# jdm365/SuffixArray

Measured on AMD Instinct MI355X. Metric: sa_build_chars_per_s, higher is better.
Workload: dtype u8 text / u32 narrow keys / u32 suffix indices / i64 output

## Files before the change

suffixarray_amd/csrc/radix_narrow.hpp:

```cpp
#pragma once
#include "radix_sort.hpp"
#include <vector>

namespace sa {

constexpr int NARROW_MAX_PASSES = 6;
constexpr int SEG_ITEMS = 24;

struct SegPlan {
    u32 bstart[RADIX + 1];
    u32 tprefix[RADIX + 1];
    u32 cfirst[NCHUNK + 1];
};

__global__ __launch_bounds__(256) void seg_plan_kernel(const u32* __restrict__ hist_top, u32 tile, SegPlan* __restrict__ plan) {
    __shared__ u32 s_w[2][4];
    __shared__ u32 s_tp[RADIX + 1];
    const int d = threadIdx.x, lane = d & 63, w = d >> 6;
    u32 size = 0;
#pragma unroll
    for (int c = 0; c < NCHUNK; ++c) size += hist_top[c * RADIX + d];
    const u32 tiles = (u32)(((u64)size + tile - 1) / tile);
    u32 is = size, it = tiles;
#pragma unroll
// ... 767 lines not shown
    __syncthreads();
#pragma unroll
    for (int k = 0; k < ITEMS; ++k) {
        const u32 p = k * BLOCK + tid;
        if (FULL || p < tile_n) a.vals_out[gidx[k]] = s_vals[p];
    }
}

template <int BLOCK>
__global__ __launch_bounds__(BLOCK, 4) void text_low_pass_kernel(TextLowArgs t) {
    constexpr int WAVES = BLOCK / WAVE;
    constexpr u32 TILE = BLOCK * SORT_ITEMS;
    constexpr int WH = (WAVES * RADIX > NCHUNK * RADIX) ? WAVES * RADIX : NCHUNK * RADIX;
    static_assert(TILE * 8 >= TILE + TEXT_HALO, "the staged codes fit the key array's LDS");
    __shared__ __attribute__((aligned(16))) u64 s_keys[TILE];
    __shared__ u32 s_whist[WH];
    __shared__ uint2 s_tab[RADIX];
    __shared__ u32 s_wsum[RADIX / WAVE];
    __shared__ u8 s_map[256];
    __shared__ u32 s_tile;
    __shared__ u32 s_chunk;
    const SortPassArgs& a = t.p;
    const int tid = threadIdx.x;
    if (tid == 0) {
        u32 tile = 0xFFFFFFFFu, chunk = 0;
        const u32 home = xcc_id();
        for (int k = 0; k < NCHUNK; ++k) {
            const u32 c = (home + k) & (NCHUNK - 1);
            const u32 first = c * a.g.tpc;
            if (first >= a.g.tiles) continue;
            const u32 cnt = (a.g.tiles - first) < a.g.tpc ? (a.g.tiles - first) : a.g.tpc;
            const u32 x = atomicAdd(&a.ticket[c], 1u);
            if (x < cnt) { tile = first + x; chunk = c; break; }
        }
        s_tile = tile;
        s_chunk = chunk;
    }
    if (tid < 256) s_map[tid] = (u8)t.map[tid];
    for (int i = tid; i < WAVES * RADIX; i += BLOCK) s_whist[i] = 0;
    __syncthreads();
    const u32 tile = s_tile;
    if (tile == 0xFFFFFFFFu) return;
    const u32 chunk = s_chunk;
    const u64 rest = t.n - (u64)tile * TILE;
    if (rest >= (u64)TILE)
        text_low_tile<true, BLOCK>(t, tile, chunk, TILE, s_keys, s_whist, s_tab, s_wsum, s_map);
    else
        text_low_tile<false, BLOCK>(t, tile, chunk, (u32)rest, s_keys, s_whist, s_tab, s_wsum, s_map);
}

struct NarrowWorkspace {
    SegPlan* plan = nullptr;
    u32* hist = nullptr;
    u32* base = nullptr;
    u32* tickets = nullptr;
    u16* map_dev = nullptr;
    CodeMap map_host;
    bool split_enabled = true;
    bool split_used = false;
    u32 split_max_seen = 0;
    u32* split_hist = nullptr;
    u32* split_base = nullptr;
    u32* split_cursor = nullptr;
    u32* top_cursor = nullptr;
    bool cursor_pad = true;
    bool split_cursor_t = false;
    bool top_atomic_ranks = false;
    bool top_claims = true;
    bool split_atomic = true;
    u32* split_sub = nullptr;
    u64* split_status = nullptr;
    u32 split_tiles = 0;
    u32 split_epoch = 0;
    u32* host_word = nullptr;
    static size_t split_table_bytes() { return (size_t)RADIX * SPLIT_NB * sizeof(u32); }
    static size_t split_sub_words() { return ((size_t)RADIX << SPLIT_BITS) + 1; }
    u32* split_levels_dev() const { return split_sub + split_sub_words(); }
    u32 split_cap = LOCAL_CAP;
    int split_rb = 0;
    int local_bin_bits = 12;
    bool split_flags = true;
    bool local_big = false;
    bool split_big = false;
    bool split_flags_done = false;
    int split_items = 28;
    static size_t hist_bytes() { return (size_t)NARROW_MAX_PASSES * RADIX * RADIX * sizeof(u32); }
    int init() {
        SA_HIP_CHECK(hipMalloc(&plan, sizeof(SegPlan)));
        SA_HIP_CHECK(hipMalloc(&hist, hist_bytes()));
        SA_HIP_CHECK(hipMalloc(&base, (size_t)RADIX * RADIX * sizeof(u32)));
        SA_HIP_CHECK(hipMalloc(&tickets, (size_t)NARROW_MAX_PASSES * NCHUNK * sizeof(u32)));
        SA_HIP_CHECK(hipMalloc(&map_dev, sizeof(CodeMap)));
        SA_HIP_CHECK(hipMalloc(&split_hist, split_table_bytes()));
        SA_HIP_CHECK(hipMalloc(&split_base, split_table_bytes()));
        SA_HIP_CHECK(hipMalloc(&split_cursor, split_table_bytes()));
        SA_HIP_CHECK(hipMalloc(&top_cursor, (size_t)RADIX * 64 * sizeof(u32)));
        SA_HIP_CHECK(hipMalloc(&split_sub, (split_sub_words() + 16) * sizeof(u32)));
        SA_HIP_CHECK(hipHostMalloc(reinterpret_cast<void**>(&host_word), 64, hipHostMallocDefault));
        if (const char* e = diag_env("SA_HIP_SPLIT")) split_enabled = atoi(e) != 0;
        if (const char* e = diag_env("SA_HIP_CURSOR_PAD")) cursor_pad = atoi(e) != 0;
        if (const char* e = diag_env("SA_HIP_SPLIT_CURSOR_T")) split_cursor_t = atoi(e) != 0;
        if (const char* e = diag_env("SA_HIP_TOP_CLAIMS")) top_claims = atoi(e) != 0;
        if (const char* e = diag_env("SA_HIP_TOP_ARANKS")) top_atomic_ranks = atoi(e) != 0;
        if (const char* e = diag_env("SA_HIP_LOCAL_BIG")) local_big = atoi(e) != 0;
        if (const char* e = diag_env("SA_HIP_SPLIT_ATOMIC")) split_atomic = atoi(e) != 0;
        if (const char* e = diag_env("SA_HIP_SPLIT_FLAGS")) split_flags = atoi(e) != 0;
        if (const char* e = diag_env("SA_HIP_LOCAL_BINS")) local_bin_bits = (atoi(e) == 11) ? 11 : 12;
        if (const char* e = diag_env("SA_HIP_SPLIT_ITEMS")) { const int v = atoi(e); split_items = (v == 24 || v == 28) ? v : 32; }
        if (const char* e = diag_env("SA_HIP_SPLIT_CAP")) { const int v = atoi(e); if (v >= 64 && v <= (int)LOCAL_CAP) split_cap = (u32)v; }
        return 0;
    }
    int ensure_split_status(u32 tiles, hipStream_t stream) {
        if (tiles <= split_tiles) return 0;
        if (split_status) { SA_HIP_CHECK(hipStreamSynchronize(stream)); (void)hipFree(split_status); }
        split_status = nullptr; split_tiles = 0;
        SA_HIP_CHECK(hipMalloc(&split_status, (size_t)tiles * SPLIT_NB * sizeof(u64)));
        SA_HIP_CHECK(hipMemsetAsync(split_status, 0, (size_t)tiles * SPLIT_NB * sizeof(u64), stream));
        split_tiles = tiles;
        return 0;
    }
    void destroy() {
        if (plan) (void)hipFree(plan);
        if (hist) (void)hipFree(hist);
        if (base) (void)hipFree(base);
        if (tickets) (void)hipFree(tickets);
        if (map_dev) (void)hipFree(map_dev);
        if (split_hist) (void)hipFree(split_hist);
        if (split_base) (void)hipFree(split_base);
        if (split_cursor) (void)hipFree(split_cursor);
        if (top_cursor) (void)hipFree(top_cursor);
        if (split_sub) (void)hipFree(split_sub);
        if (split_status) (void)hipFree(split_status);
        if (host_word) (void)hipHostFree(host_word);
        map_dev = nullptr;
        plan = nullptr; hist = nullptr; base = nullptr; tickets = nullptr;
        split_hist = split_base = split_sub = split_cursor = top_cursor = nullptr; split_status = nullptr; split_tiles = 0; host_word = nullptr;
    }
};

inline bool narrow_sort_applies(const RadixWorkspace& ws, u64 n, int begin_bit) {
    return ws.block == 512 && begin_bit >= 24 && begin_bit < 56 && n >= (1u << 22) &&
           n / ws.tile() + RADIX + 1 <= ws.max_tiles;
}

struct TextSource {
    const u8* text;
    int b, k0;
};
inline bool text_pass_applies(int b, int k0) { return b <= 8 && k0 - 1 <= TEXT_HALO; }

inline int narrow_text_histogram(RadixWorkspace& ws, NarrowWorkspace& nw, hipStream_t stream, const u8* text, const CodeMap& map,
                                 u32 n, int b) {
    nw.map_host = map;
    SA_HIP_CHECK(hipMemcpyAsync(nw.map_dev, nw.map_host.code, sizeof(CodeMap), hipMemcpyHostToDevice, stream));
    const SortGeom g = make_geom(n, TEXT_TILE);
    const u32 spans = div_up(n, 4096);
    const dim3 grid(spans < 2048u ? spans : 2048u), block(256);
    switch ((8 + b - 1) / b) {
        case 1: hipLaunchKernelGGL(top_hist_kernel<1>, grid, block, 0, stream, text, nw.map_dev, (u64)n, b, g, ws.hist(0)); break;
        case 2: hipLaunchKernelGGL(top_hist_kernel<2>, grid, block, 0, stream, text, nw.map_dev, (u64)n, b, g, ws.hist(0)); break;
        case 3: hipLaunchKernelGGL(top_hist_kernel<3>, grid, block, 0, stream, text, nw.map_dev, (u64)n, b, g, ws.hist(0)); break;
        case 4: hipLaunchKernelGGL(top_hist_kernel<4>, grid, block, 0, stream, text, nw.map_dev, (u64)n, b, g, ws.hist(0)); break;
        default: hipLaunchKernelGGL(top_hist_kernel<8>, grid, block, 0, stream, text, nw.map_dev, (u64)n, b, g, ws.hist(0)); break;
    }
    return 0;
}

inline int wide_text_histogram(RadixWorkspace& ws, NarrowWorkspace& nw, hipStream_t stream, const u8* text, const CodeMap& map,
                               u32 n, int b, int k0) {
    nw.map_host = map;
    SA_HIP_CHECK(hipMemcpyAsync(nw.map_dev, nw.map_host.code, sizeof(CodeMap), hipMemcpyHostToDevice, stream));
    const SortGeom g = make_geom(n, ws.tile());
    const u32 spans = div_up(n, 4096);
    const dim3 grid(spans < 2048u ? spans : 2048u), block(256);
    switch ((8 + b - 1) / b) {
        case 1: hipLaunchKernelGGL(top_hist_kernel<1>, grid, block, 0, stream, text, nw.map_dev, (u64)n, b, g, ws.hist(0), k0); break;
        case 2: hipLaunchKernelGGL(top_hist_kernel<2>, grid, block, 0, stream, text, nw.map_dev, (u64)n, b, g, ws.hist(0), k0); break;
        case 3: hipLaunchKernelGGL(top_hist_kernel<3>, grid, block, 0, stream, text, nw.map_dev, (u64)n, b, g, ws.hist(0), k0); break;
        case 4: hipLaunchKernelGGL(top_hist_kernel<4>, grid, block, 0, stream, text, nw.map_dev, (u64)n, b, g, ws.hist(0), k0); break;
        default: hipLaunchKernelGGL(top_hist_kernel<8>, grid, block, 0, stream, text, nw.map_dev, (u64)n, b, g, ws.hist(0), k0); break;
    }
    return 0;
}
struct WideTextCtx {
    const u8* text;
    const u16* map;
    u64 n;
// ... 60 lines not shown
    const u32 split_flat_max = n / split_tile_n + 1 + RADIX;
    hipLaunchKernelGGL(seg_plan_kernel, dim3(1), dim3(256), 0, stream, ws.hist(0), try_split ? split_tile_n : seg_tile_n, nw.plan);
    nw.split_used = false;
    nw.split_flags_done = false;
    nw.split_max_seen = 0;
    if (try_split) {
        const int hb = (lo_bits - LOCAL_BIN_BITS < SPLIT_BITS) ? lo_bits - LOCAL_BIN_BITS : SPLIT_BITS;
        SA_HIP_CHECK(hipMemsetAsync(nw.split_hist, 0, NarrowWorkspace::split_table_bytes(), stream));
        SA_HIP_CHECK(hipMemsetAsync(nw.split_levels_dev(), 0, 16 * sizeof(u32), stream));
        const u32 tpb = 4;
        if (nw.split_items == 32)
            hipLaunchKernelGGL((split_hist_kernel<512, 32>), dim3(div_up(split_flat_max, tpb)), dim3(512), 0, stream,
                               reinterpret_cast<const u32*>(keysB), nw.plan, lo_bits - hb, (1u << hb) - 1u, nw.split_hist, tpb);
        else if (nw.split_items == 28)
            hipLaunchKernelGGL((split_hist_kernel<512, 28>), dim3(div_up(split_flat_max, tpb)), dim3(512), 0, stream,
                               reinterpret_cast<const u32*>(keysB), nw.plan, lo_bits - hb, (1u << hb) - 1u, nw.split_hist, tpb);
        else
            hipLaunchKernelGGL((split_hist_kernel<512, 24>), dim3(div_up(split_flat_max, tpb)), dim3(512), 0, stream,
                               reinterpret_cast<const u32*>(keysB), nw.plan, lo_bits - hb, (1u << hb) - 1u, nw.split_hist, tpb);
        hipLaunchKernelGGL(split_levels_kernel, dim3(RADIX), dim3(SPLIT_NB), 0, stream, (const u32*)nw.split_hist, hb, nw.split_levels_dev());
        SA_HIP_CHECK(hipMemcpyAsync(nw.host_word, nw.split_levels_dev(), 16 * sizeof(u32), hipMemcpyDeviceToHost, stream));
        SA_HIP_CHECK(hipStreamSynchronize(stream));
        int rb = -1;
        bool big = nw.local_big;
        if (!big)
            for (int k = 1; k <= hb; ++k)
                if (nw.host_word[k] <= nw.split_cap) { rb = k; break; }
        if (rb < 0 && nw.split_cap == LOCAL_CAP) {
            for (int k = 1; k <= hb; ++k)
                if (nw.host_word[k] <= LOCAL_CAP_BIG && lo_bits - k >= 12) { rb = k; big = true; break; }
            if (rb < 0) big = false;
        }
        nw.split_max_seen = nw.host_word[rb > 0 ? rb : hb];
        if (rb > 0) {
            const int rest_bits = lo_bits - rb;
            const int dshift = lo_bits - rb;
            const u32 dmask = (1u << rb) - 1u;
            hipLaunchKernelGGL(split_scan_kernel, dim3(RADIX), dim3(SPLIT_NB), 0, stream, (const u32*)nw.split_hist, nw.plan, hb, rb,
                               nw.split_base, nw.split_sub);
            if (!nw.split_atomic && (rc = nw.ensure_split_status(split_flat_max, stream))) return rc;
            if (nw.split_atomic) SA_HIP_CHECK(hipMemsetAsync(nw.split_cursor, 0, NarrowWorkspace::split_table_bytes(), stream));
            if (++ws.epoch >= (1u << 30)) {
                SA_HIP_CHECK(hipMemsetAsync(ws.status, 0, (size_t)ws.max_tiles * RADIX * sizeof(u64), stream));
                ws.epoch = 1;
            }
            if (!nw.split_atomic && ws.epoch <= nw.split_epoch)
                SA_HIP_CHECK(hipMemsetAsync(nw.split_status, 0, (size_t)nw.split_tiles * SPLIT_NB * sizeof(u64), stream));
            nw.split_epoch = ws.epoch;
            SplitPassArgs a;
            a.keys_in = reinterpret_cast<const u32*>(keysB); a.vals_in = valsB;
            a.keys_out = reinterpret_cast<u32*>(keysA); a.vals_out = valsA;
            a.plan = nw.plan; a.shift = dshift; a.mask = dmask; a.digit_base = nw.split_base; a.status = nw.split_status;
            a.ticket = nw.tickets; a.epoch = ws.epoch; a.dstat = ws.dstat; a.incl_mask = SA_INCL_MASK; a.cursor = nw.split_cursor;
            a.cur_bs = nw.split_cursor_t ? 1u : (u32)SPLIT_NB; a.cur_ds = nw.split_cursor_t ? (u32)RADIX : 1u;
            if ((rc = ws.timer.start(stream, 2))) return rc;
            if (nw.split_atomic) {
                if (nw.split_items == 32) hipLaunchKernelGGL((seg_split_kernel<512, 32, true>), dim3(split_flat_max), dim3(512), 0, stream, a);
                else if (nw.split_items == 28) hipLaunchKernelGGL((seg_split_kernel<512, 28, true>), dim3(split_flat_max), dim3(512), 0, stream, a);
                else hipLaunchKernelGGL((seg_split_kernel<512, 24, true>), dim3(split_flat_max), dim3(512), 0, stream, a);
            } else {
                if (nw.split_items == 32) hipLaunchKernelGGL((seg_split_kernel<512, 32, false>), dim3(split_flat_max), dim3(512), 0, stream, a);
                else if (nw.split_items == 28) hipLaunchKernelGGL((seg_split_kernel<512, 28, false>), dim3(split_flat_max), dim3(512), 0, stream, a);
                else hipLaunchKernelGGL((seg_split_kernel<512, 24, false>), dim3(split_flat_max), dim3(512), 0, stream, a);
            }
            if ((rc = ws.timer.stop(stream, (u64)n * 16u))) return rc;
            ws.pass_records += n; ws.pass_bytes += (u64)n * 16u; ws.passes += 1;
            LocalArgs l;
            l.keys_in = reinterpret_cast<const u32*>(keysA); l.vals_in = valsA;
            l.keys_out = reinterpret_cast<u32*>(keysB); l.vals_out = valsB; l.vals_out64 = vals_res64;
            l.sub = nw.split_sub;
            const int bb = (big || (rest_bits >= 12 && nw.local_bin_bits == 12)) ? 12 : 11;
            l.bin_shift = rest_bits - bb;
            l.dstat = ws.dstat;
            const u64 local_bytes = (u64)n * 16u + (vals_res64 ? (u64)n * 8u : 0u);
            nw.split_flags_done = false;
            l.dir = DirArgs{}; l.counts = nullptr; l.lite = LiteArgs{}; l.lo_shift = begin_bit; l.rb = rb; l.n = n;
            bool with_flags = false;
            if (nw.split_flags && flags_req && flags_req->prepare) {
                const int fr = flags_req->prepare(flags_req->ctx, (u32)RADIX << rb, &l);
                if (fr < 0) return fr;
                with_flags = (fr == 0) && l.dir.dir && l.dir.dbits >= 8 + rb && l.dir.dbits - 8 - rb <= bb && l.dir.dbits - 8 <= lo_bits;
            }
            if ((rc = ws.timer.start(stream, 3))) return rc;
            const dim3 lgrid((u32)RADIX << rb), lblock(big ? LOCAL_BLOCK_BIG : LOCAL_BLOCK);
            if (big) {
                if (with_flags) hipLaunchKernelGGL((local_finish_kernel<12, true, LOCAL_BLOCK_BIG>), lgrid, lblock, 0, stream, l);
                else hipLaunchKernelGGL((local_finish_kernel<12, false, LOCAL_BLOCK_BIG>), lgrid, lblock, 0, stream, l);
            } else if (with_flags) {
                if (bb == 12) hipLaunchKernelGGL((local_finish_kernel<12, true>), lgrid, lblock, 0, stream, l);
                else hipLaunchKernelGGL((local_finish_kernel<11, true>), lgrid, lblock, 0, stream, l);
            } else {
                if (bb == 12) hipLaunchKernelGGL((local_finish_kernel<12, false>), lgrid, lblock, 0, stream, l);
                else hipLaunchKernelGGL((local_finish_kernel<11, false>), lgrid, lblock, 0, stream, l);
            }
            nw.split_flags_done = with_flags;
            nw.split_big = big;
            if ((rc = ws.timer.stop(stream, local_bytes))) return rc;
            ws.pass_records += n; ws.pass_bytes += local_bytes; ws.passes += 1;
            SA_HIP_CHECK(hipGetLastError());
            if (diag_env("SA_HIP_SPLIT_DEBUG")) {
                const u32 nsub = (u32)RADIX << rb;
                std::vector<u32> sub(nsub + 1), k1(n), k2(n), v2(n), bst(RADIX + 1);
                SA_HIP_CHECK(hipStreamSynchronize(stream));
                SA_HIP_CHECK(hipMemcpy(sub.data(), nw.split_sub, (size_t)(nsub + 1) * 4, hipMemcpyDeviceToHost));
                SA_HIP_CHECK(hipMemcpy(k1.data(), keysA, (size_t)n * 4, hipMemcpyDeviceToHost));
                SA_HIP_CHECK(hipMemcpy(k2.data(), keysB, (size_t)n * 4, hipMemcpyDeviceToHost));
                SA_HIP_CHECK(hipMemcpy(v2.data(), valsB, (size_t)n * 4, hipMemcpyDeviceToHost));
                SA_HIP_CHECK(hipMemcpy(bst.data(), nw.plan->bstart, (size_t)(RADIX + 1) * 4, hipMemcpyDeviceToHost));
                u64 bad_sub = 0, bad_split = 0, bad_sorted = 0, bad_mono = 0;
                u32 first_split = ~0u, first_sorted = ~0u;
                for (u32 i = 0; i < nsub; ++i) {
                    if (sub[i] > sub[i + 1] || sub[i + 1] > n) { ++bad_mono; continue; }
                    if ((i & (((u32)1 << rb) - 1)) == 0 && sub[i] != bst[i >> rb]) ++bad_sub;
                    for (u32 j = sub[i]; j < sub[i + 1]; ++j) {
                        if (((k1[j] >> dshift) & dmask) != (i & dmask)) { ++bad_split; if (first_split == ~0u) first_split = j; }
                        if (j > sub[i] && (k2[j - 1] > k2[j] || (k2[j - 1] == k2[j] && v2[j - 1] >= v2[j]))) { ++bad_sorted; if (first_sorted == ~0u) first_sorted = j; }
                    }
                }
                fprintf(stderr, "[sa_hip] split debug: n=%u rb=%d hb=%d nsub=%u sub[0]=%u sub[last]=%u | table: %llu not monotone, %llu off the bucket starts | split pass: %llu records in the wrong group (first %u) | local pass: %llu out of order (first %u)\n",
                        n, rb, hb, nsub, sub[0], sub[nsub], (unsigned long long)bad_mono, (unsigned long long)bad_sub, (unsigned long long)bad_split, first_split,
                        (unsigned long long)bad_sorted, first_sorted);
            }
            nw.split_used = true;
            nw.split_rb = rb;
            *keys_res = reinterpret_cast<u64*>(keysB);
            *vals_res = valsB;
            return 0;
        }
    }
    if (optimistic) {
        SA_HIP_CHECK(hipMemsetAsync(ws.tickets(), 0, NCHUNK * sizeof(u32), stream));
        if (++ws.epoch >= (1u << 30)) {
            SA_HIP_CHECK(hipMemsetAsync(ws.status, 0, (size_t)ws.max_tiles * RADIX * sizeof(u64), stream));
            ws.epoch = 1;
        }
        if ((rc = launch_text_top(false))) return rc;
    }
    if (try_split && split_tile_n != seg_tile_n)
        hipLaunchKernelGGL(seg_plan_kernel, dim3(1), dim3(256), 0, stream, ws.hist(0), seg_tile_n, nw.plan);
    SA_HIP_CHECK(hipMemsetAsync(nw.hist, 0, NarrowWorkspace::hist_bytes(), stream));
    {
        const u32 tpb = 4;
        const u32 mask0 = (1u << ((np == 1) ? lo_bits : RADIX_BITS)) - 1u;
        hipLaunchKernelGGL((seg_hist_kernel<512, SEG_ITEMS>), dim3(div_up(flat_max, tpb)), dim3(512), 0, stream,
                           reinterpret_cast<const u32*>(keysB), nw.plan, 0, mask0, nw.hist, tpb);
    }
    u32* kin = reinterpret_cast<u32*>(keysB); u32* vin = valsB;
    u32* kout = reinterpret_cast<u32*>(keysA); u32* vout = valsA;
    for (int p = 0; p < np; ++p) {
        if (++ws.epoch >= (1u << 30)) {
            SA_HIP_CHECK(hipMemsetAsync(ws.status, 0, (size_t)ws.max_tiles * RADIX * sizeof(u64), stream));
            ws.epoch = 1;
        }
        const bool last = (p == np - 1);
        const int bits_p = last ? (lo_bits - RADIX_BITS * (np - 1)) : RADIX_BITS;
        hipLaunchKernelGGL(seg_scan_kernel, dim3(RADIX), dim3(256), 0, stream, nw.hist + (size_t)p * RADIX * RADIX, nw.plan, nw.base);
        SegPassArgs a;
        a.keys_in = kin; a.vals_in = vin; a.keys_out = kout; a.keys_out64 = keep_narrow ? nullptr : reinterpret_cast<u64*>(kout);
        a.vals_out = vout;
        a.vals_out64 = last ? vals_res64 : nullptr;
        a.plan = nw.plan;
        a.shift = RADIX_BITS * p;
        a.mask = (1u << bits_p) - 1u;
        a.next_shift = last ? -1 : RADIX_BITS * (p + 1);
        const int bits_n = (p + 1 == np - 1) ? (lo_bits - RADIX_BITS * (np - 1)) : RADIX_BITS;
        a.next_mask = last ? 0u : ((1u << bits_n) - 1u);
        a.digit_base = nw.base;
        a.next_hist = last ? nullptr : nw.hist + (size_t)(p + 1) * RADIX * RADIX;
// ... 19 lines not shown
```

suffixarray_amd/csrc/radix_split.hpp:

```cpp
#pragma once
#include "flags_common.hpp"

namespace sa {

#ifndef SA_ABL
#define SA_ABL 0
#endif
constexpr int SPLIT_BITS = 10;
constexpr int SPLIT_NB = 1 << SPLIT_BITS;
constexpr u32 LOCAL_CAP = 8192;
constexpr int LOCAL_BLOCK = 512;
constexpr int LOCAL_ITEMS = (int)(LOCAL_CAP / LOCAL_BLOCK);
constexpr u32 LOCAL_CAP_BIG = 16384;
constexpr int LOCAL_BLOCK_BIG = 1024;
constexpr int LOCAL_BIN_BITS = 11;
constexpr int SPLIT_HIST_COPIES = 4;

template <int BLOCK, int ITEMS>
__global__ __launch_bounds__(BLOCK) void split_hist_kernel(const u32* __restrict__ keys, const SegPlan* __restrict__ plan, int shift,
                                                           u32 mask, u32* __restrict__ hist, u32 tiles_per_block) {
    constexpr u32 TILE = BLOCK * ITEMS;
    constexpr int CS = SPLIT_NB + 1;
    __shared__ u32 s_h[SPLIT_HIST_COPIES * CS];
    __shared__ u32 s_t[RADIX + 1];
    for (int i = threadIdx.x; i <= RADIX; i += BLOCK) s_t[i] = plan->tprefix[i];
    for (int i = threadIdx.x; i < SPLIT_HIST_COPIES * CS; i += BLOCK) s_h[i] = 0;
    __syncthreads();
    const u32 F = s_t[RADIX];
    const u32 f_lo = blockIdx.x * tiles_per_block;
    const u32 f_hi = (f_lo + tiles_per_block < F) ? f_lo + tiles_per_block : F;
    if (f_lo >= f_hi) return;
    u32* my = s_h + (threadIdx.x & (SPLIT_HIST_COPIES - 1)) * CS;
    auto flush = [&](u32 bucket) {
        sync_lds();
        for (int d = threadIdx.x; d < SPLIT_NB; d += BLOCK) {
            u32 v = 0;
#pragma unroll
            for (int k = 0; k < SPLIT_HIST_COPIES; ++k) { v += s_h[k * CS + d]; s_h[k * CS + d] = 0; }
            if (v) atomicAdd(&hist[bucket * SPLIT_NB + d], v);
        }
        sync_lds();
    };
    u32 cur = seg_bucket_of(s_t, f_lo);
    for (u32 f = f_lo; f < f_hi; ++f) {
        const u32 b = seg_bucket_of(s_t, f);
        if (b != cur) { flush(cur); cur = b; }
        const u32 start = plan->bstart[b] + ((f - s_t[b]) * TILE);
        const u32 end = plan->bstart[b + 1];
        const u32 len = (end - start) < TILE ? (end - start) : TILE;
        if (len == TILE) {
            u32 k[ITEMS];
#pragma unroll
            for (int j = 0; j < ITEMS; ++j) k[j] = keys[start + j * BLOCK + threadIdx.x];
#pragma unroll
            for (int j = 0; j < ITEMS; ++j) atomicAdd(&my[(k[j] >> shift) & mask], 1u);
        } else {
            for (u32 l = threadIdx.x; l < len; l += BLOCK) atomicAdd(&my[(keys[start + l] >> shift) & mask], 1u);
        }
    }
    flush(cur);
}

__global__ __launch_bounds__(SPLIT_NB) void split_levels_kernel(const u32* __restrict__ hist, int hb, u32* __restrict__ levels) {
    __shared__ u32 s_p[SPLIT_NB + 1];
    __shared__ u32 s_w[SPLIT_NB / WAVE];
    const int b = blockIdx.x, d = threadIdx.x, lane = d & 63, w = d >> 6;
    const u32 c = hist[b * SPLIT_NB + d];
    u32 incl = c;
#pragma unroll
    for (int o = 1; o < 64; o <<= 1) {
        const u32 t = __shfl_up(incl, o);
        if (lane >= o) incl += t;
    }
    if (lane == 63) s_w[w] = incl;
    __syncthreads();
    for (int i = 0; i < w; ++i) incl += s_w[i];
    s_p[d + 1] = incl;
    if (d == 0) s_p[0] = 0;
    __syncthreads();
    __shared__ u32 s_lv[SPLIT_BITS + 1][SPLIT_NB / WAVE];
    for (int k = 0; k <= hb; ++k) {
        const int g = hb - k;
        u32 v = 0;
        if (d < (1 << k)) v = s_p[(d + 1) << g] - s_p[d << g];
#pragma unroll
        for (int o = 32; o > 0; o >>= 1) { const u32 t = __shfl_down(v, o); v = t > v ? t : v; }
        if (lane == 0) s_lv[k][w] = v;
    }
    __syncthreads();
    if (d <= hb) {
        u32 v = 0;
        for (int i = 0; i < SPLIT_NB / WAVE; ++i) v = s_lv[d][i] > v ? s_lv[d][i] : v;
        if (v) atomicMax(&levels[d], v);
    }
}

__global__ __launch_bounds__(SPLIT_NB) void split_scan_kernel(const u32* __restrict__ hist, const SegPlan* __restrict__ plan, int hb, int rb,
// ... 183 lines not shown
        const u32 p = woff + j * WAVE;
        val[j] = (FULL || p < tile_n) ? vin[p] : 0u;
    }
    __syncthreads();
    u32* s_vals = s_keys;
#pragma unroll
    for (int j = 0; j < ITEMS; ++j)
        if (FULL || (woff + j * WAVE) < tile_n) s_vals[(pp[j >> 1] >> ((j & 1) * 16)) & 0xFFFFu] = val[j];
    __syncthreads();
#pragma unroll
    for (int k = 0; k < ITEMS; ++k) {
        const u32 p = k * BLOCK + tid;
        if (FULL || p < tile_n) a.vals_out[gidx[k]] = s_vals[p];
    }
}

template <int BLOCK, int ITEMS, bool ATOMIC>
__global__ __launch_bounds__(BLOCK, 4) void seg_split_kernel(SplitPassArgs a) {
    constexpr u32 TILE = BLOCK * ITEMS;
    __shared__ __attribute__((aligned(16))) u32 s_keys[TILE];
    __shared__ __attribute__((aligned(16))) u32 s_cnt[SPLIT_NB + 4];
    __shared__ __attribute__((aligned(16))) u32 s_gdelta[SPLIT_NB];
    __shared__ u32 s_wsum[BLOCK / WAVE];
    __shared__ u32 s_t[RADIX + 1];
    __shared__ u32 s_b[RADIX + 1];
    __shared__ u32 s_c[NCHUNK + 1];
    __shared__ u32 s_flat;

    const int tid = threadIdx.x;
    u32 home = 0, t_home = 0;
    if (tid == 0) {
        home = xcc_id();
        t_home = atomicAdd(&a.ticket[home], 1u);
    }
    for (int i = tid; i <= RADIX; i += BLOCK) { s_t[i] = a.plan->tprefix[i]; s_b[i] = a.plan->bstart[i]; }
    if (tid <= NCHUNK) s_c[tid] = a.plan->cfirst[tid];
    for (int i = tid; i < SPLIT_NB + 4; i += BLOCK) s_cnt[i] = 0;
    __syncthreads();
    if (tid == 0) {
        u32 flat = 0xFFFFFFFFu;
        if (t_home < s_c[home + 1] - s_c[home]) flat = s_c[home] + t_home;
        for (int k = 1; k < NCHUNK && flat == 0xFFFFFFFFu; ++k) {
            const u32 c = (home + k) & (NCHUNK - 1);
            const u32 cnt = s_c[c + 1] - s_c[c];
            if (cnt == 0) continue;
            const u32 t = atomicAdd(&a.ticket[c], 1u);
            if (t < cnt) flat = s_c[c] + t;
        }
        s_flat = flat;
    }
    __syncthreads();
    const u32 flat = s_flat;
    if (flat == 0xFFFFFFFFu) return;
    const u32 bucket = seg_bucket_of(s_t, flat);
    const u32 first_flat = s_t[bucket];
    const u32 start = s_b[bucket] + (flat - first_flat) * TILE;
    const u32 rest = s_b[bucket + 1] - start;
    if (rest >= TILE) split_tile<true, BLOCK, ITEMS, ATOMIC>(a, flat, first_flat, bucket, start, TILE, s_keys, s_cnt, s_gdelta, s_wsum);
    else split_tile<false, BLOCK, ITEMS, ATOMIC>(a, flat, first_flat, bucket, start, rest, s_keys, s_cnt, s_gdelta, s_wsum);
}

struct LocalArgs {
    const u32* keys_in;
    const u32* vals_in;
    u32* keys_out;
    u32* vals_out;
    int64_t* vals_out64;
    const u32* sub;
    int bin_shift;
    DeviceStatus* dstat;
    DirArgs dir;
    uint2* counts;
    LiteArgs lite;
    int lo_shift;
    int rb;
    u32 n;
};

struct LocalFlagsRequest {
    int (*prepare)(void* ctx, u32 nsub, LocalArgs* l) = nullptr;
    void* ctx = nullptr;
};

template <int BB, bool FLAGS, int BLOCK = LOCAL_BLOCK>
__global__ __launch_bounds__(BLOCK, 4) void local_finish_kernel(LocalArgs a) {
    constexpr int ITEMS = LOCAL_ITEMS;
    constexpr u32 CAP = (u32)BLOCK * ITEMS;
    constexpr int NB = 1 << BB, WORDS = NB / 2, WPT = WORDS / BLOCK;
    static_assert(WPT >= 1 && WPT * BLOCK == WORDS, "the scan covers the counters exactly");
    static_assert(CAP < 65536, "16-bit counters and starts");
    __shared__ __attribute__((aligned(16))) u64 s_rec[CAP + 2];
    __shared__ __attribute__((aligned(16))) u32 s_cw[WORDS + 4];
    __shared__ u32 s_wsum[BLOCK / WAVE];
    const int tid = threadIdx.x, lane = tid & 63, wave = tid >> 6;
    const u32 s = a.sub[blockIdx.x];
    const u32 m = a.sub[blockIdx.x + 1] - s;
    const int g2 = FLAGS ? a.dir.dbits - 8 - a.rb : 0;
    const u32 dfirst = FLAGS ? (blockIdx.x << g2) : 0u;
    const u32 nd = FLAGS ? (1u << g2) : 0u;
    if (FLAGS && tid == 0 && blockIdx.x == gridDim.x - 1) a.dir.dir[1u << a.dir.dbits] = a.n;
    if (m == 0) {
        if (FLAGS) {
            if (!(SA_ABL & 8)) for (u32 e = tid; e < nd; e += BLOCK) a.dir.dir[dfirst + e] = s;
        }
        return;
    }
    if (m > CAP) {
        if (tid == 0) __hip_atomic_store(&a.dstat->error, 1u, __ATOMIC_RELAXED, __HIP_MEMORY_SCOPE_AGENT);
        return;
    }
    const u32* kin = a.keys_in + s;
    const u32* vin = a.vals_in + s;
    if (!FLAGS && m == 1) {
        if (tid == 0) {
            const u32 k = kin[0], v = vin[0];
            a.keys_out[s] = k; a.vals_out[s] = v;
            if (a.vals_out64) a.vals_out64[s] = (int64_t)v;
        }
        return;
    }
#pragma unroll
    for (int i = 0; i < WPT; ++i) s_cw[WPT * tid + i] = 0;
    __syncthreads();

    u32 key[ITEMS], val[ITEMS], r[ITEMS];
#pragma unroll
    for (int j = 0; j < ITEMS; ++j) {
        const u32 p = (u32)j * BLOCK + tid;
        key[j] = 0; val[j] = 0;
        if ((u32)j * BLOCK < m && p < m) { key[j] = kin[p]; val[j] = vin[p]; }
    }
#pragma unroll
    for (int j = 0; j < ITEMS; ++j) {
        const u32 p = (u32)j * BLOCK + tid;
        r[j] = 0;
        if ((u32)j * BLOCK < m && p < m) {
            const u32 b = (key[j] >> a.bin_shift) & (u32)(NB - 1);
            const u32 sh = (b & 1u) * 16u;
            r[j] = (atomicAdd(&s_cw[b >> 1], 1u << sh) >> sh) & 0xFFFFu;
        }
    }
    sync_lds();

    {
        u32 cw[WPT];
        u32 tot = 0;
#pragma unroll
        for (int i = 0; i < WPT; ++i) { cw[i] = s_cw[WPT * tid + i]; tot += (cw[i] & 0xFFFFu) + (cw[i] >> 16); }
        u32 incl = tot;
#pragma unroll
        for (int o = 1; o < 64; o <<= 1) {
            const u32 t = __shfl_up(incl, o);
            if (lane >= o) incl += t;
        }
        if (lane == 63) s_wsum[wave] = incl;
        __syncthreads();
        u32 run = incl - tot;
        for (int i = 0; i < wave; ++i) run += s_wsum[i];
#pragma unroll
        for (int i = 0; i < WPT; ++i) {
            const u32 c0 = cw[i] & 0xFFFFu, c1 = cw[i] >> 16;
            s_cw[WPT * tid + i] = run | ((run + c0) << 16);
            run += c0 + c1;
        }
        if (tid == BLOCK - 1) s_cw[WORDS] = m;
    }
    __syncthreads();
    const u16* s_st = reinterpret_cast<const u16*>(s_cw);

#pragma unroll
    for (int j = 0; j < ITEMS; ++j) {
        const u32 p = (u32)j * BLOCK + tid;
        if ((u32)j * BLOCK < m && p < m) {
            const u32 slot = (u32)s_st[(key[j] >> a.bin_shift) & (u32)(NB - 1)] + r[j];
            s_rec[slot] = ((u64)key[j] << 32) | (u64)val[j];
        }
    }
    __syncthreads();

    u64 rec[ITEMS];
#pragma unroll
    for (int j = 0; j < ITEMS; ++j) {
        const u32 p = (u32)j * BLOCK + tid;
        rec[j] = 0; r[j] = 0;
        if ((u32)j * BLOCK < m && p < m) {
            const u64 x = s_rec[p];
            const u32 bin = ((u32)(x >> 32) >> a.bin_shift) & (u32)(NB - 1);
            const u32 lo = s_st[bin], hi = s_st[bin + 1];
            u32 cnt = 0;
            for (u32 q = lo; q < hi; q += 2) {
                const u64 y0 = s_rec[q], y1 = s_rec[q + 1];
                cnt += (y0 < x) ? 1u : 0u;
                cnt += (q + 1 < hi && y1 < x) ? 1u : 0u;
            }
            rec[j] = x;
            r[j] = lo + cnt;
        }
    }
    __syncthreads();
#pragma unroll
    for (int j = 0; j < ITEMS; ++j) {
        const u32 p = (u32)j * BLOCK + tid;
        if ((u32)j * BLOCK < m && p < m) s_rec[r[j]] = rec[j];
    }
    if (FLAGS && tid == 0) s_rec[m] = ~0ull;
    __syncthreads();

    auto stage_pair = [&](u32 p) {
        const u64 x = s_rec[p], xn = s_rec[p + 1];
        const bool starts = (p == 0) || ((u32)(s_rec[p - 1] >> 32) != (u32)(x >> 32));
        u32 at = atomicAdd(&a.counts[blockIdx.x].x, starts ? 2u : 1u);
        if (at + (starts ? 2u : 1u) > LITE_CAP) __hip_atomic_store(a.lite.overflow, 1u, __ATOMIC_RELAXED, __HIP_MEMORY_SCOPE_AGENT);
        if (starts) {
            atomicAdd(&a.counts[blockIdx.x].y, 1u);
            if (at < LITE_CAP) {
                const u64 row = (u64)blockIdx.x * LITE_CAP + at;
                a.lite.st_pos[row] = s + p; a.lite.st_idx[row] = (u32)x; a.lite.st_head[row] = 1;
            }
            ++at;
        }
        if (at < LITE_CAP) {
            const u64 row = (u64)blockIdx.x * LITE_CAP + at;
            a.lite.st_pos[row] = s + p + 1; a.lite.st_idx[row] = (u32)xn; a.lite.st_head[row] = 0;
        }
    };
    if (FLAGS) {
        if (!(SA_ABL & 1)) for (u32 e = tid; e < nd; e += BLOCK) a.dir.dir[dfirst + e] = s + (u32)s_st[e << (BB - g2)];
        if (!(SA_ABL & 4))
        for (u32 p = (u32)tid * 16u + 15u; p + 1 < m; p += (u32)BLOCK * 16u)
            if ((u32)(s_rec[p] >> 32) == (u32)(s_rec[p + 1] >> 32)) stage_pair(p);
    }
    u32 tmask = 0;
#pragma unroll
    for (int j = 0; j < ITEMS; ++j) {
        const u32 p = (u32)j * BLOCK + tid;
        if ((u32)j * BLOCK < m) {
            const u64 x = s_rec[p];
            const u32 k = (u32)(x >> 32);
            if (p < m) {
                a.keys_out[s + p] = k;
                a.vals_out[s + p] = (u32)x;
                if (a.vals_out64) a.vals_out64[s + p] = (int64_t)(u32)x;
            }
            if (FLAGS && !(SA_ABL & 2)) {
                const u32 kn = (u32)__builtin_amdgcn_update_dpp((int)~k, (int)k, 0x101, 0xF, 0xF, false);
                tmask |= (kn == k && p + 1 < m) ? (1u << j) : 0u;
            }
        }
    }
    if (FLAGS) {
        while (tmask) {
            const u32 j = (u32)__builtin_ctz(tmask);
            tmask &= tmask - 1u;
            stage_pair(j * BLOCK + (u32)tid);
        }
    }
}

}
```

Baseline: 72.04 billion.

## Add persistent local-finish kernel with ticketed sub-bucket runs and prefetch

Result: faster. 76.79 billion (median of 6 runs) (+6.6%).

```diff
diff --git a/suffixarray_amd/csrc/radix_narrow.hpp b/suffixarray_amd/csrc/radix_narrow.hpp
--- a/suffixarray_amd/csrc/radix_narrow.hpp
+++ b/suffixarray_amd/csrc/radix_narrow.hpp
@@ -873,6 +873,22 @@
     bool split_flags = true;
     bool local_big = false;
     bool split_big = false;
+    bool local_persist = true;
+    u32 local_grid_force = 0;
+    u32 local_grid[6] = {};
+    template <typename K>
+    int persist_grid(K kernel, int block, int slot, u32 nsub, u32* grid) {
+        if (!local_grid[slot]) {
+            int dev = 0, cus = 0, per_cu = 0;
+            SA_HIP_CHECK(hipGetDevice(&dev));
+            SA_HIP_CHECK(hipDeviceGetAttribute(&cus, hipDeviceAttributeMultiprocessorCount, dev));
+            SA_HIP_CHECK(hipOccupancyMaxActiveBlocksPerMultiprocessor(&per_cu, reinterpret_cast<const void*>(kernel), block, 0));
+            local_grid[slot] = (u32)((per_cu > 0 ? per_cu : 1) * (cus > 0 ? cus : 1));
+        }
+        const u32 g = local_grid_force ? local_grid_force : local_grid[slot];
+        *grid = g < nsub ? g : nsub;
+        return 0;
+    }
     bool split_flags_done = false;
     int split_items = 28;
     static size_t hist_bytes() { return (size_t)NARROW_MAX_PASSES * RADIX * RADIX * sizeof(u32); }
@@ -894,6 +910,8 @@
         if (const char* e = diag_env("SA_HIP_TOP_CLAIMS")) top_claims = atoi(e) != 0;
         if (const char* e = diag_env("SA_HIP_TOP_ARANKS")) top_atomic_ranks = atoi(e) != 0;
         if (const char* e = diag_env("SA_HIP_LOCAL_BIG")) local_big = atoi(e) != 0;
+        if (const char* e = diag_env("SA_HIP_LOCAL_PERSIST")) local_persist = atoi(e) != 0;
+        if (const char* e = diag_env("SA_HIP_LOCAL_GRID")) { const int v = atoi(e); local_grid_force = v > 0 ? (u32)v : 0u; }
         if (const char* e = diag_env("SA_HIP_SPLIT_ATOMIC")) split_atomic = atoi(e) != 0;
         if (const char* e = diag_env("SA_HIP_SPLIT_FLAGS")) split_flags = atoi(e) != 0;
         if (const char* e = diag_env("SA_HIP_LOCAL_BINS")) local_bin_bits = (atoi(e) == 11) ? 11 : 12;
@@ -1120,8 +1138,21 @@
                 with_flags = (fr == 0) && l.dir.dir && l.dir.dbits >= 8 + rb && l.dir.dbits - 8 - rb <= bb && l.dir.dbits - 8 <= lo_bits;
             }
             if ((rc = ws.timer.start(stream, 3))) return rc;
-            const dim3 lgrid((u32)RADIX << rb), lblock(big ? LOCAL_BLOCK_BIG : LOCAL_BLOCK);
-            if (big) {
+            const u32 nsub = (u32)RADIX << rb;
+            const dim3 lgrid(nsub), lblock(big ? LOCAL_BLOCK_BIG : LOCAL_BLOCK);
+            if (nw.local_persist) {
+                const int slot = big ? (with_flags ? 0 : 1) : 2 + (with_flags ? 0 : 1) + (bb == 12 ? 0 : 2);
+                u32 pg = 0;
+                auto go = [&](auto kernel) -> int {
+                    if ((rc = nw.persist_grid(kernel, (int)lblock.x, slot, nsub, &pg))) return rc;
+                    hipLaunchKernelGGL(kernel, dim3(pg), lblock, 0, stream, l, (const u32*)nw.split_sub, nsub, nw.tickets + NCHUNK, LOCAL_RUN);
+                    return 0;
+                };
+                if (big) rc = with_flags ? go(local_persist_kernel<12, true, LOCAL_BLOCK_BIG>) : go(local_persist_kernel<12, false, LOCAL_BLOCK_BIG>);
+                else if (with_flags) rc = (bb == 12) ? go(local_persist_kernel<12, true>) : go(local_persist_kernel<11, true>);
+                else rc = (bb == 12) ? go(local_persist_kernel<12, false>) : go(local_persist_kernel<11, false>);
+                if (rc) return rc;
+            } else if (big) {
                 if (with_flags) hipLaunchKernelGGL((local_finish_kernel<12, true, LOCAL_BLOCK_BIG>), lgrid, lblock, 0, stream, l);
                 else hipLaunchKernelGGL((local_finish_kernel<12, false, LOCAL_BLOCK_BIG>), lgrid, lblock, 0, stream, l);
             } else if (with_flags) {
diff --git a/suffixarray_amd/csrc/radix_split.hpp b/suffixarray_amd/csrc/radix_split.hpp
--- a/suffixarray_amd/csrc/radix_split.hpp
+++ b/suffixarray_amd/csrc/radix_split.hpp
@@ -13,6 +13,7 @@
 constexpr int LOCAL_ITEMS = (int)(LOCAL_CAP / LOCAL_BLOCK);
 constexpr u32 LOCAL_CAP_BIG = 16384;
 constexpr int LOCAL_BLOCK_BIG = 1024;
+constexpr u32 LOCAL_RUN = 8;
 constexpr int LOCAL_BIN_BITS = 11;
 constexpr int SPLIT_HIST_COPIES = 4;
 
@@ -362,54 +363,17 @@
     void* ctx = nullptr;
 };
 
-template <int BB, bool FLAGS, int BLOCK = LOCAL_BLOCK>
-__global__ __launch_bounds__(BLOCK, 4) void local_finish_kernel(LocalArgs a) {
+template <int BB, bool FLAGS, int BLOCK, bool PERSIST, typename Mid>
+__device__ __forceinline__ void local_finish_sub(const LocalArgs& a, const u32 sb, const u32 s, const u32 m, u32 (&key)[LOCAL_ITEMS],
+                                                 u32 (&val)[LOCAL_ITEMS], u64* s_rec, u32* s_cw, u32* s_wsum, Mid&& mid) {
     constexpr int ITEMS = LOCAL_ITEMS;
-    constexpr u32 CAP = (u32)BLOCK * ITEMS;
     constexpr int NB = 1 << BB, WORDS = NB / 2, WPT = WORDS / BLOCK;
-    static_assert(WPT >= 1 && WPT * BLOCK == WORDS, "the scan covers the counters exactly");
-    static_assert(CAP < 65536, "16-bit counters and starts");
-    __shared__ __attribute__((aligned(16))) u64 s_rec[CAP + 2];
-    __shared__ __attribute__((aligned(16))) u32 s_cw[WORDS + 4];
-    __shared__ u32 s_wsum[BLOCK / WAVE];
     const int tid = threadIdx.x, lane = tid & 63, wave = tid >> 6;
-    const u32 s = a.sub[blockIdx.x];
-    const u32 m = a.sub[blockIdx.x + 1] - s;
     const int g2 = FLAGS ? a.dir.dbits - 8 - a.rb : 0;
-    const u32 dfirst = FLAGS ? (blockIdx.x << g2) : 0u;
+    const u32 dfirst = FLAGS ? (sb << g2) : 0u;
     const u32 nd = FLAGS ? (1u << g2) : 0u;
-    if (FLAGS && tid == 0 && blockIdx.x == gridDim.x - 1) a.dir.dir[1u << a.dir.dbits] = a.n;
-    if (m == 0) {
-        if (FLAGS) {
-            if (!(SA_ABL & 8)) for (u32 e = tid; e < nd; e += BLOCK) a.dir.dir[dfirst + e] = s;
-        }
-        return;
-    }
-    if (m > CAP) {
-        if (tid == 0) __hip_atomic_store(&a.dstat->error, 1u, __ATOMIC_RELAXED, __HIP_MEMORY_SCOPE_AGENT);
-        return;
-    }
-    const u32* kin = a.keys_in + s;
-    const u32* vin = a.vals_in + s;
-    if (!FLAGS && m == 1) {
-        if (tid == 0) {
-            const u32 k = kin[0], v = vin[0];
-            a.keys_out[s] = k; a.vals_out[s] = v;
-            if (a.vals_out64) a.vals_out64[s] = (int64_t)v;
-        }
-        return;
-    }
-#pragma unroll
-    for (int i = 0; i < WPT; ++i) s_cw[WPT * tid + i] = 0;
-    __syncthreads();
-
-    u32 key[ITEMS], val[ITEMS], r[ITEMS];
-#pragma unroll
-    for (int j = 0; j < ITEMS; ++j) {
-        const u32 p = (u32)j * BLOCK + tid;
-        key[j] = 0; val[j] = 0;
-        if ((u32)j * BLOCK < m && p < m) { key[j] = kin[p]; val[j] = vin[p]; }
-    }
+
+    u32 r[ITEMS];
 #pragma unroll
     for (int j = 0; j < ITEMS; ++j) {
         const u32 p = (u32)j * BLOCK + tid;
@@ -457,6 +421,7 @@
         }
     }
     __syncthreads();
+    if (FLAGS && !(SA_ABL & 1)) for (u32 e = tid; e < nd; e += BLOCK) a.dir.dir[dfirst + e] = s + (u32)s_st[e << (BB - g2)];
 
     u64 rec[ITEMS];
 #pragma unroll
@@ -478,34 +443,38 @@
         }
     }
     __syncthreads();
+    if (PERSIST) {
+#pragma unroll
+        for (int i = 0; i < WPT; ++i) s_cw[WPT * tid + i] = 0;
+    }
 #pragma unroll
     for (int j = 0; j < ITEMS; ++j) {
         const u32 p = (u32)j * BLOCK + tid;
         if ((u32)j * BLOCK < m && p < m) s_rec[r[j]] = rec[j];
     }
-    if (FLAGS && tid == 0) s_rec[m] = ~0ull;
-    __syncthreads();
+    if (FLAGS && tid == 0) { const u64 ones = ~(u64)(m >> 31); s_rec[m] = ones; }
+    __syncthreads();
+    mid();
 
     auto stage_pair = [&](u32 p) {
         const u64 x = s_rec[p], xn = s_rec[p + 1];
         const bool starts = (p == 0) || ((u32)(s_rec[p - 1] >> 32) != (u32)(x >> 32));
-        u32 at = atomicAdd(&a.counts[blockIdx.x].x, starts ? 2u : 1u);
+        u32 at = atomicAdd(&a.counts[sb].x, starts ? 2u : 1u);
         if (at + (starts ? 2u : 1u) > LITE_CAP) __hip_atomic_store(a.lite.overflow, 1u, __ATOMIC_RELAXED, __HIP_MEMORY_SCOPE_AGENT);
         if (starts) {
-            atomicAdd(&a.counts[blockIdx.x].y, 1u);
+            atomicAdd(&a.counts[sb].y, 1u);
             if (at < LITE_CAP) {
-                const u64 row = (u64)blockIdx.x * LITE_CAP + at;
+                const u64 row = (u64)sb * LITE_CAP + at;
                 a.lite.st_pos[row] = s + p; a.lite.st_idx[row] = (u32)x; a.lite.st_head[row] = 1;
             }
             ++at;
         }
         if (at < LITE_CAP) {
-            const u64 row = (u64)blockIdx.x * LITE_CAP + at;
+            const u64 row = (u64)sb * LITE_CAP + at;
             a.lite.st_pos[row] = s + p + 1; a.lite.st_idx[row] = (u32)xn; a.lite.st_head[row] = 0;
         }
     };
     if (FLAGS) {
-        if (!(SA_ABL & 1)) for (u32 e = tid; e < nd; e += BLOCK) a.dir.dir[dfirst + e] = s + (u32)s_st[e << (BB - g2)];
         if (!(SA_ABL & 4))
         for (u32 p = (u32)tid * 16u + 15u; p + 1 < m; p += (u32)BLOCK * 16u)
             if ((u32)(s_rec[p] >> 32) == (u32)(s_rec[p + 1] >> 32)) stage_pair(p);
@@ -537,4 +506,147 @@
     }
 }
 
-}
+template <int BLOCK>
+__device__ __forceinline__ void local_load(const LocalArgs& a, const u32 s, const u32 m, u32 (&key)[LOCAL_ITEMS], u32 (&val)[LOCAL_ITEMS]) {
+    const u32* kin = a.keys_in + s;
+    const u32* vin = a.vals_in + s;
+#pragma unroll
+    for (int j = 0; j < LOCAL_ITEMS; ++j) {
+        const u32 p = (u32)j * BLOCK + threadIdx.x;
+        key[j] = 0; val[j] = 0;
+        if ((u32)j * BLOCK < m && p < m) { key[j] = kin[p]; val[j] = vin[p]; }
+    }
+}
+
+template <bool FLAGS, int BLOCK>
+__device__ __forceinline__ bool local_short_sub(const LocalArgs& a, const u32 sb, const u32 s, const u32 m, const u32 cap) {
+    if (m == 0) {
+        if (FLAGS && !(SA_ABL & 8)) {
+            const int g2 = a.dir.dbits - 8 - a.rb;
+            const u32 dfirst = sb << g2, nd = 1u << g2;
+            for (u32 e = threadIdx.x; e < nd; e += BLOCK) a.dir.dir[dfirst + e] = s;
+        }
+        return true;
+    }
+    if (m > cap) {
+        if (threadIdx.x == 0) __hip_atomic_store(&a.dstat->error, 1u, __ATOMIC_RELAXED, __HIP_MEMORY_SCOPE_AGENT);
+        return true;
+    }
+    if (!FLAGS && m == 1) {
+        if (threadIdx.x == 0) {
+            const u32 k = a.keys_in[s], v = a.vals_in[s];
+            a.keys_out[s] = k; a.vals_out[s] = v;
+            if (a.vals_out64) a.vals_out64[s] = (int64_t)v;
+        }
+        return true;
+    }
+    return false;
+}
+
+template <int BB, bool FLAGS, int BLOCK = LOCAL_BLOCK>
+__global__ __launch_bounds__(BLOCK, 4) void local_finish_kernel(LocalArgs a) {
+    constexpr u32 CAP = (u32)BLOCK * LOCAL_ITEMS;
+    constexpr int NB = 1 << BB, WORDS = NB / 2, WPT = WORDS / BLOCK;
+    static_assert(WPT >= 1 && WPT * BLOCK == WORDS, "the scan covers the counters exactly");
+    static_assert(CAP < 65536, "16-bit counters and starts");
+    __shared__ __attribute__((aligned(16))) u64 s_rec[CAP + 2];
+    __shared__ __attribute__((aligned(16))) u32 s_cw[WORDS + 4];
+    __shared__ u32 s_wsum[BLOCK / WAVE];
+    const u32 sb = blockIdx.x;
+    const u32 s = a.sub[sb];
+    const u32 m = a.sub[sb + 1] - s;
+    if (FLAGS && threadIdx.x == 0 && sb == gridDim.x - 1) a.dir.dir[1u << a.dir.dbits] = a.n;
+    if (local_short_sub<FLAGS, BLOCK>(a, sb, s, m, CAP)) return;
+#pragma unroll
+    for (int i = 0; i < WPT; ++i) s_cw[WPT * threadIdx.x + i] = 0;
+    __syncthreads();
+    u32 key[LOCAL_ITEMS], val[LOCAL_ITEMS];
+    local_load<BLOCK>(a, s, m, key, val);
+    local_finish_sub<BB, FLAGS, BLOCK, false>(a, sb, s, m, key, val, s_rec, s_cw, s_wsum, [] {});
+}
+
+__device__ __forceinline__ u32 wave_lower_bound(const u32* __restrict__ sub, const u32 nsub, const u64 t) {
+    const u32 lane = threadIdx.x & 63u;
+    u32 lo = 0, hi = nsub;
+    while (lo < hi) {
+        const u32 step = (hi - lo + 63u) / 64u;
+        const u32 i = lo + lane * step;
+        const u32 c = (u32)__popcll(__ballot(i < hi && (u64)sub[i] < t));
+        if (c == 0) break;
+        const u32 nlo = lo + (c - 1u) * step + 1u;
+        hi = (lo + c * step < hi) ? lo + c * step : hi;
+        lo = nlo;
+    }
+    return lo;
+}
+
+template <int BB, bool FLAGS, int BLOCK = LOCAL_BLOCK>
+__global__ __launch_bounds__(BLOCK, 4) void local_persist_kernel(LocalArgs a, const u32* __restrict__ sub, u32 nsub, u32* ticket, u32 run) {
+    constexpr u32 CAP = (u32)BLOCK * LOCAL_ITEMS;
+    constexpr int NB = 1 << BB, WORDS = NB / 2, WPT = WORDS / BLOCK;
+    static_assert(WPT >= 1 && WPT * BLOCK == WORDS, "the scan covers the counters exactly");
+    static_assert(CAP < 65536, "16-bit counters and starts");
+    static_assert(BLOCK >= (NCHUNK - 1) * WAVE, "a wave per region bound");
+    __shared__ __attribute__((aligned(16))) u64 s_rec[CAP + 2];
+    __shared__ __attribute__((aligned(16))) u32 s_cw[WORDS + 4];
+    __shared__ u32 s_wsum[BLOCK / WAVE];
+    __shared__ u32 s_reg[NCHUNK + 1];
+    __shared__ u32 s_run[2];
+    const int tid = threadIdx.x;
+    {
+        const u32 v = (u32)(tid >> 6);
+        if (v + 1 < (u32)NCHUNK) {
+            const u32 b = wave_lower_bound(sub, nsub, (u64)(v + 1) * sub[nsub] / NCHUNK);
+            if ((tid & 63) == 0) s_reg[v + 1] = b;
+        }
+        if (tid == 0) { s_reg[0] = 0; s_reg[NCHUNK] = nsub; }
+    }
+#pragma unroll
+    for (int i = 0; i < WPT; ++i) s_cw[WPT * tid + i] = 0;
+    __syncthreads();
+    const u32 home = xcc_id() & (NCHUNK - 1);
+    u32 lo = 0, hi = 0;
+    auto grab = [&] {
+        if (tid == 0) {
+            u32 r0 = 0, r1 = 0;
+            for (int k = 0; k < NCHUNK; ++k) {
+                const u32 c = (home + (u32)k) & (NCHUNK - 1);
+                const u32 b0 = s_reg[c], b1 = s_reg[c + 1];
+                if (b0 >= b1) continue;
+                const u64 st = (u64)b0 + (u64)atomicAdd(&ticket[c], 1u) * run;
+                if (st < b1) { r0 = (u32)st; r1 = (st + run < b1) ? (u32)(st + run) : b1; break; }
+            }
+            s_run[0] = r0; s_run[1] = r1;
+        }
+        __syncthreads();
+        lo = __builtin_amdgcn_readfirstlane(s_run[0]);
+        hi = __builtin_amdgcn_readfirstlane(s_run[1]);
+        __syncthreads();
+    };
+    auto next = [&](u32 i, u32& s, u32& m) -> u32 {
+        for (;; ++i) {
+            if (i >= hi) {
+                grab();
+                if (lo >= hi) return nsub;
+                i = lo;
+            }
+            s = sub[i]; m = sub[i + 1] - s;
+            if (FLAGS && tid == 0 && i == nsub - 1) a.dir.dir[1u << a.dir.dbits] = a.n;
+            if (!local_short_sub<FLAGS, BLOCK>(a, i, s, m, CAP)) return i;
+        }
+    };
+    u32 key[LOCAL_ITEMS], val[LOCAL_ITEMS];
+    u32 s = 0, m = 0;
+    u32 i = next(0, s, m);
+    if (i < nsub) local_load<BLOCK>(a, s, m, key, val);
+    while (i < nsub) {
+        u32 ns = 0, nm = 0;
+        const u32 nx = next(i + 1, ns, nm);
+        local_finish_sub<BB, FLAGS, BLOCK, true>(a, i, s, m, key, val, s_rec, s_cw, s_wsum, [&] {
+            if (nx < nsub) local_load<BLOCK>(a, ns, nm, key, val);
+        });
+        i = nx; s = ns; m = nm;
+    }
+}
+
+}
```
